# Daniel-Starr/pointcloudhookup

Hardware: AMD Instinct MI355X
Metric: Mpts/s ground-filter+tower-cluster, 100 M-pt corridor; % HBM roofline on kNN (higher is better)
Workload: dtype f32 (filter) + f64 (distance predicate)

## Files before the change

pointcloudhookup_amd/csrc/pch_dbscan.hip:

```cpp
#include <assert.h>
#include "pch_prims.h"

namespace pch {

constexpr int DB_THREADS = 256;
constexpr int DB_WAVES   = DB_THREADS / 64;
constexpr int DB_ROWS    = 25;
constexpr int INT_BIG    = 0x7fffffff;
constexpr int DB_FEW_QUERIES = 24;
constexpr int DB_AHEAD = 3;
constexpr long long DB_LONG_TOT = 8192;
constexpr int DB_SEGS = 43;

struct DbGrid {
    float   ox, oy, oz;
    double  cell;
    double  inv_cell;
    double  eps2;
    float   eps2_lo, eps2_hi;
    int     bx, by, bz;
    int     mx, my, mz;
    int64_t chunk_size;
    const uint32_t* chunk_bad;
    const uint32_t* chunk_cells;
    int     min_samples;
};

__constant__ int8_t DB_ROW_DY[DB_ROWS] = {0, 1, -1, 0, 0, 1, 1, -1, -1, 2, -2, 0, 0,
                                          2, 2, -2, -2, 1, 1, -1, -1, 2, 2, -2, -2};
__constant__ int8_t DB_ROW_DZ[DB_ROWS] = {0, 0, 0, 1, -1, 1, -1, 1, -1, 0, 0, 2, -2,
                                          1, -1, 1, -1, 2, -2, 2, -2, 2, -2, 2, -2};

__device__ __forceinline__ uint64_t db_pack(const DbGrid& g, uint64_t chunk, uint64_t cz,
                                            uint64_t cy, uint64_t cx) {
    return ((((chunk << g.bz) | cz) << g.by | cy) << g.bx) | cx;
}

__device__ __forceinline__ bool db_within(const float4& q, const float4& p, double eps2) {
    const double dx = (double)q.x - (double)p.x;
    const double dy = (double)q.y - (double)p.y;
    const double dz = (double)q.z - (double)p.z;
    double d = dx * dx;
    d += dy * dy;
    d += dz * dz;
    return d <= eps2;
}

__device__ __forceinline__ bool db_within2(const float4& q, const float4& p, const DbGrid& g) {
    const float dx = q.x - p.x, dy = q.y - p.y, dz = q.z - p.z;
    float d = dx * dx;
    d = __builtin_fmaf(dy, dy, d);
    d = __builtin_fmaf(dz, dz, d);
    if (d <= g.eps2_lo) return true;
    if (d >= g.eps2_hi) return false;
    return db_within(q, p, g.eps2);
}

typedef float f32x2 __attribute__((ext_vector_type(2)));
struct __attribute__((aligned(16))) DbPair { f32x2 x, y, z, pad; };

__device__ __forceinline__ void db_tile_put(DbPair* __restrict__ tile, int l, const float4& p) {
    float* f = reinterpret_cast<float*>(&tile[l >> 1]);
    f[l & 1] = p.x; f[2 + (l & 1)] = p.y; f[4 + (l & 1)] = p.z;
}
__device__ __forceinline__ float4 db_tile_get(const DbPair* __restrict__ tile, int k) {
    const float* f = reinterpret_cast<const float*>(&tile[k >> 1]);
    float4 p;
    p.x = f[k & 1]; p.y = f[2 + (k & 1)]; p.z = f[4 + (k & 1)]; p.w = 0.0f;
    return p;
}
__device__ __forceinline__ int db_tile_count(const float4& q, const DbPair* __restrict__ tile, int nj,
                                             const DbGrid& g) {
    const f32x2 qx = {q.x, q.x}, qy = {q.y, q.y}, qz = {q.z, q.z};
    const float lo = g.eps2_lo, hi = g.eps2_hi;
    int c_lo = 0, c_hi = 0;
    const int np = ((nj + 7) & ~7) >> 1;
    for (int k = 0; k < np; k += 4) {
        f32x2 px[4], py[4], pz[4];
#pragma unroll
        for (int u = 0; u < 4; ++u) { px[u] = tile[k + u].x; py[u] = tile[k + u].y; pz[u] = tile[k + u].z; }
#pragma unroll
        for (int u = 0; u < 4; ++u) {
            const f32x2 dx = qx - px[u], dy = qy - py[u], dz = qz - pz[u];
            f32x2 d = dx * dx;
            d = __builtin_elementwise_fma(dy, dy, d);
            d = __builtin_elementwise_fma(dz, dz, d);
            c_lo += (d.x <= lo ? 1 : 0) + (d.y <= lo ? 1 : 0);
            c_hi += (d.x < hi ? 1 : 0) + (d.y < hi ? 1 : 0);
        }
    }
    if (c_lo != c_hi) {
        c_lo = 0;
        for (int k = 0; k < nj; ++k) c_lo += db_within2(q, db_tile_get(tile, k), g) ? 1 : 0;
    }
    return c_lo;
}

__device__ __forceinline__ double db_box_d2(const float4& q, const float* __restrict__ box) {
    const double gx = fmax(fmax((double)box[0] - (double)q.x, (double)q.x - (double)box[3]), 0.0);
    const double gy = fmax(fmax((double)box[1] - (double)q.y, (double)q.y - (double)box[4]), 0.0);
    const double gz = fmax(fmax((double)box[2] - (double)q.z, (double)q.z - (double)box[5]), 0.0);
    double d = gx * gx;
    d += gy * gy;
    d += gz * gz;
    return d;
}
__device__ __forceinline__ double db_boxbox_d2(const float* __restrict__ a, const float* __restrict__ b) {
    const double gx = fmax(fmax((double)b[0] - (double)a[3], (double)a[0] - (double)b[3]), 0.0);
    const double gy = fmax(fmax((double)b[1] - (double)a[4], (double)a[1] - (double)b[4]), 0.0);
    const double gz = fmax(fmax((double)b[2] - (double)a[5], (double)a[2] - (double)b[5]), 0.0);
    double d = gx * gx;
    d += gy * gy;
    d += gz * gz;
    return d;
}

__device__ __forceinline__ bool db_row_bad(const float* __restrict__ xyz, int64_t i) {
    const uint32_t a = __float_as_uint(xyz[3 * i + 0]) & 0x7FFFFFFFu;
    const uint32_t b = __float_as_uint(xyz[3 * i + 1]) & 0x7FFFFFFFu;
    const uint32_t c = __float_as_uint(xyz[3 * i + 2]) & 0x7FFFFFFFu;
    return a >= 0x7F800000u || b >= 0x7F800000u || c >= 0x7F800000u;
}
__global__ __launch_bounds__(DB_THREADS) void db_chunkbad_k(const float* __restrict__ xyz, int64_t n,
                                                            int64_t chunk_size, uint32_t* __restrict__ bad) {
    for (int64_t i = (int64_t)blockIdx.x * DB_THREADS + threadIdx.x; i < n;
         i += (int64_t)gridDim.x * DB_THREADS)
        if (db_row_bad(xyz, i)) atomicOr(&bad[i / chunk_size], 1u);
}

__global__ __launch_bounds__(DB_THREADS) void db_first_bad_k(const float* __restrict__ xyz, int64_t n,
                                                             unsigned long long* __restrict__ first) {
    unsigned long long best = ~0ull;
    for (int64_t i = (int64_t)blockIdx.x * DB_THREADS + threadIdx.x; i < n;
         i += (int64_t)gridDim.x * DB_THREADS)
        if (db_row_bad(xyz, i) && (unsigned long long)i < best) best = (unsigned long long)i;
    best = wave_reduce_min(best);
    if (lane_id() == 0 && best != ~0ull) atomicMin(first, best);
}

__global__ __launch_bounds__(DB_THREADS) void db_aabb_in_k(const float* __restrict__ xyz, int64_t n,
                                                           uint32_t* __restrict__ mm) {
    uint32_t lo[3] = {0xFFFFFFFFu, 0xFFFFFFFFu, 0xFFFFFFFFu}, hi[3] = {0u, 0u, 0u};
    for (int64_t i = (int64_t)blockIdx.x * DB_THREADS + threadIdx.x; i < n;
         i += (int64_t)gridDim.x * DB_THREADS) {
        const float x = xyz[3 * i + 0], y = xyz[3 * i + 1], z = xyz[3 * i + 2];
        if (!(fabsf(x) < INFINITY && fabsf(y) < INFINITY && fabsf(z) < INFINITY)) continue;
        const float v[3] = {x, y, z};
#pragma unroll
        for (int a = 0; a < 3; ++a) {
            const uint32_t k = f32_ordered(v[a]);
            lo[a] = k < lo[a] ? k : lo[a];
            hi[a] = k > hi[a] ? k : hi[a];
        }
    }
#pragma unroll
    for (int a = 0; a < 3; ++a) {
        lo[a] = wave_reduce_min(lo[a]);
        hi[a] = wave_reduce_max(hi[a]);
        if (lane_id() == 0) {
            if (lo[a] != 0xFFFFFFFFu) atomicMin(&mm[a], lo[a]);
            if (hi[a] != 0u) atomicMax(&mm[3 + a], hi[a]);
        }
    }
}

__device__ __forceinline__ bool db_cell_coords(const DbGrid& g, float x, float y, float z,
                                               uint32_t& cx, uint32_t& cy, uint32_t& cz) {
    const double fx = floor(((double)x - (double)g.ox) * g.inv_cell);
    const double fy = floor(((double)y - (double)g.oy) * g.inv_cell);
    const double fz = floor(((double)z - (double)g.oz) * g.inv_cell);
    const bool ok = fx >= 0.0 && fx <= (double)g.mx && fy >= 0.0 && fy <= (double)g.my &&
                    fz >= 0.0 && fz <= (double)g.mz;
    cx = ok ? (uint32_t)fx : 0u; cy = ok ? (uint32_t)fy : 0u; cz = ok ? (uint32_t)fz : 0u;
    return ok;
}

__global__ __launch_bounds__(DB_THREADS) void db_keys_k(const float* __restrict__ xyz, int64_t n,
                                                        DbGrid g, const uint32_t* __restrict__ bad,
                                                        uint64_t* __restrict__ keys,
                                                        uint32_t* __restrict__ vals,
                                                        uint32_t* __restrict__ status) {
    const int64_t i = (int64_t)blockIdx.x * DB_THREADS + threadIdx.x;
    if (i >= n) return;
    vals[i] = (uint32_t)i;
    if (bad[i / g.chunk_size]) {
        keys[i] = db_pack(g, (uint64_t)(i / g.chunk_size), 0, 0, 0);
        return;
    }
    const float x = xyz[3 * i + 0], y = xyz[3 * i + 1], z = xyz[3 * i + 2];
    uint32_t cx, cy, cz;
    if (!db_cell_coords(g, x, y, z, cx, cy, cz)) atomicOr(status, 1u);
    keys[i] = db_pack(g, (uint64_t)(i / g.chunk_size), cz, cy, cx);
}

__global__ __launch_bounds__(DB_THREADS) void dbc_axis_keys_k(const float* __restrict__ xyz, int64_t n, int axis,
                                                              uint64_t* __restrict__ keys, uint32_t* __restrict__ vals) {
    const int64_t i = (int64_t)blockIdx.x * DB_THREADS + threadIdx.x;
    if (i >= n) return;
    keys[i] = f32_ordered(xyz[3 * i + axis]);
    vals[i] = (uint32_t)i;
}
__global__ __launch_bounds__(DB_THREADS) void dbc_heads_k(const uint64_t* __restrict__ keys, int64_t n, double inv_cell,
                                                          uint32_t* __restrict__ head) {
    const int64_t i = (int64_t)blockIdx.x * DB_THREADS + threadIdx.x;
    if (i >= n) return;
    bool h = i == 0;
    if (i > 0) {
        const double a = (double)f32_unordered((uint32_t)keys[i - 1]), b = (double)f32_unordered((uint32_t)keys[i]);
        h = (b - a) * inv_cell >= 3.0;
    }
    head[i] = h ? 1u : 0u;
}
__global__ __launch_bounds__(DB_THREADS) void dbc_local_k(const uint64_t* __restrict__ keys, const uint32_t* __restrict__ flag,
                                                          const uint32_t* __restrict__ excl, int64_t n, double inv_cell,
                                                          float* __restrict__ headx, int phase,
                                                          uint32_t* __restrict__ li, uint32_t* __restrict__ seglen,
                                                          uint32_t* __restrict__ status) {
    const int64_t i = (int64_t)blockIdx.x * DB_THREADS + threadIdx.x;
    if (i >= n) return;
    const uint32_t seg = excl[i] + flag[i] - 1u;
    const float x = f32_unordered((uint32_t)keys[i]);
    if (phase == 0) {
        if (flag[i]) headx[seg] = x;
        return;
    }
    const double v = floor(((double)x - (double)headx[seg]) * inv_cell);
    uint32_t u = 0;
    if (v >= 0.0 && v < 2147483000.0) u = (uint32_t)v; else atomicOr(status, 2u);
    li[i] = u;
    const bool last = i + 1 == n || flag[i + 1] != 0u;
    if (last) seglen[seg] = u + 3u;
}
__global__ __launch_bounds__(DB_THREADS) void dbc_comp_k(const uint32_t* __restrict__ vals, const uint32_t* __restrict__ flag,
                                                         const uint32_t* __restrict__ excl, const uint32_t* __restrict__ li,
                                                         const uint32_t* __restrict__ segoff, int64_t n, int axis,
                                                         uint32_t* __restrict__ comp, uint32_t* __restrict__ cmax) {
    const int64_t i = (int64_t)blockIdx.x * DB_THREADS + threadIdx.x;
    if (i >= n) return;
    const uint32_t seg = excl[i] + flag[i] - 1u;
    const uint32_t c = segoff[seg] + li[i];
    comp[3 * (int64_t)vals[i] + axis] = c;
    if (i == n - 1) cmax[axis] = c;
}
__global__ __launch_bounds__(DB_THREADS) void db_keys_comp_k(const uint32_t* __restrict__ comp, int64_t n, DbGrid g,
                                                             uint64_t* __restrict__ keys, uint32_t* __restrict__ vals) {
    const int64_t i = (int64_t)blockIdx.x * DB_THREADS + threadIdx.x;
    if (i >= n) return;
    vals[i] = (uint32_t)i;
    keys[i] = db_pack(g, 0, comp[3 * i + 2], comp[3 * i + 1], comp[3 * i + 0]);
}
__global__ __launch_bounds__(DB_THREADS) void db_add_offset_k(int32_t* __restrict__ labels, int64_t n, int32_t off) {
    const int64_t i = (int64_t)blockIdx.x * DB_THREADS + threadIdx.x;
    if (i < n && labels[i] >= 0) labels[i] += off;
}

__global__ __launch_bounds__(DB_THREADS) void db_gather_k(const float* __restrict__ xyz,
                                                          const uint64_t* __restrict__ keys,
                                                          const uint32_t* __restrict__ vals, int64_t n,
                                                          float4* __restrict__ pts) {
    const int64_t i = (int64_t)blockIdx.x * DB_THREADS + threadIdx.x;
    if (i >= n) return;
    const uint32_t o = vals[i];
    float4 p;
    p.x = xyz[3 * (int64_t)o + 0];
    p.y = xyz[3 * (int64_t)o + 1];
    p.z = xyz[3 * (int64_t)o + 2];
    p.w = __uint_as_float(o);
    pts[i] = p;
}

struct Row3 { float x, y, z; };
constexpr int CS_THREADS = 1024;
constexpr int CS_WAVES   = CS_THREADS / 64;
constexpr int CS_ROUNDS  = 4;
constexpr int CS_TILE    = CS_THREADS * CS_ROUNDS;
constexpr int CS_PASSES  = 4;
constexpr int CS_HREP    = 4;
constexpr int CS_BINS    = 512;
constexpr int64_t CS_MAX_CHUNK = 1 << 17;
constexpr int64_t CS_MIN_CHUNKS = 96;

__device__ __forceinline__ uint32_t cs_cell_key(const DbGrid& g, float x, float y, float z, bool& ok) {
    uint32_t cx, cy, cz;
    ok = db_cell_coords(g, x, y, z, cx, cy, cz);
    return (((cz << g.by) | cy) << g.bx) | cx;
}

constexpr int CS_HU = 8;
__device__ __forceinline__ void cs_load_rows(const Row3* __restrict__ rows, int i0, int cn, Row3 (&q)[CS_HU]) {
#pragma unroll
    for (int u = 0; u < CS_HU; ++u) {
        const int i = i0 + u * CS_THREADS + (int)threadIdx.x;
        q[u] = rows[i < cn ? i : 0];
    }
}
__device__ __forceinline__ bool cs_row_check(const Row3& q, bool in, bool ok, uint32_t* flags) {
    const bool fin = fabsf(q.x) < INFINITY && fabsf(q.y) < INFINITY && fabsf(q.z) < INFINITY;
    if (in && !fin) flags[0] = 1u;
    else if (in && !ok) flags[1] = 1u;
    return fin;
}
__device__ __forceinline__ uint64_t cs_chunk_field(const DbGrid& g, int64_t c) {
    const int sh = g.bx + g.by + g.bz;
    return sh < 64 ? ((uint64_t)c << sh) : 0ull;
}
__device__ __forceinline__ void cs_rows_in_place(const DbGrid& g, const Row3* __restrict__ rows, int cn, int64_t lo,
        uint64_t hi, bool isbad, float4* __restrict__ pts, uint64_t* __restrict__ keys_out) {
    for (int i = threadIdx.x; i < cn; i += CS_THREADS) {
        const Row3 q = rows[i];
        float4 o4;
        o4.x = q.x; o4.y = q.y; o4.z = q.z; o4.w = __uint_as_float((uint32_t)(lo + i));
        pts[lo + i] = o4;
        bool ok;
        if (keys_out) keys_out[lo + i] = isbad ? hi : (hi | cs_cell_key(g, q.x, q.y, q.z, ok));
// ... 329 lines not shown
    __syncthreads();
    for (int i0 = 0; i0 < cn; i0 += CS_HU * CS_THREADS) {
        Row3 q[CS_HU];
        cs_load_rows(rows, i0, cn, q);
#pragma unroll
        for (int u = 0; u < CS_HU; ++u) {
            const int i = i0 + u * CS_THREADS + tid;
            if (i < cn) {
                bool ok;
                const uint32_t k = cs_cell_key(g, q[u].x, q[u].y, q[u].z, ok);
                uint32_t h = ct_hash(k);
                for (int p = 0; p < CT_SLOTS && tkey[h] != k; ++p) h = (h + 1u) & (CT_SLOTS - 1);
                const uint32_t pos = atomicAdd(&tcnt[h], 1u);
                if (pos >= (uint32_t)cn) continue;
                float4 o4;
                o4.x = q[u].x; o4.y = q[u].y; o4.z = q[u].z; o4.w = __uint_as_float((uint32_t)(lo + i));
                pts[lo + pos] = o4;
                if constexpr (!TABLE) keys_out[lo + pos] = hi | k;
            }
        }
    }
}

constexpr int DC_ITEMS = SCAN_TILE / DB_THREADS;
static_assert(DC_ITEMS == 8, "two 64-byte key loads per thread");

__device__ __forceinline__ void dc_load_keys(const uint64_t* __restrict__ keys, int64_t base, int64_t n,
                                             uint64_t (&k)[DC_ITEMS], uint64_t& prev) {
    if (base + DC_ITEMS <= n) {
        const ulonglong2* q = reinterpret_cast<const ulonglong2*>(keys + base);
#pragma unroll
        for (int j = 0; j < DC_ITEMS / 2; ++j) { const ulonglong2 v = q[j]; k[2 * j] = v.x; k[2 * j + 1] = v.y; }
    } else {
#pragma unroll
        for (int j = 0; j < DC_ITEMS; ++j) k[j] = base + j < n ? keys[base + j] : 0ull;
    }
    prev = (base > 0 && base < n) ? keys[base - 1] : 0ull;
}

__global__ __launch_bounds__(DB_THREADS) void db_heads_k(const uint64_t* __restrict__ keys, int64_t n,
                                                         uint32_t* __restrict__ tile_sums) {
    __shared__ uint32_t wsum[DB_WAVES];
    const int64_t base = (int64_t)blockIdx.x * SCAN_TILE + (int64_t)threadIdx.x * DC_ITEMS;
    uint64_t k[DC_ITEMS], prev;
    dc_load_keys(keys, base, n, k, prev);
    uint32_t heads = 0;
#pragma unroll
    for (int j = 0; j < DC_ITEMS; ++j) {
        const int64_t i = base + j;
        heads += (i < n && (i == 0 || k[j] != (j ? k[j - 1] : prev))) ? 1u : 0u;
    }
    heads = wave_reduce_add(heads);
    if (lane_id() == 0) wsum[wave_id()] = heads;
    __syncthreads();
    if (threadIdx.x == 0) {
        uint32_t t = 0;
#pragma unroll
        for (int w = 0; w < DB_WAVES; ++w) t += wsum[w];
        tile_sums[blockIdx.x] = t;
    }
}

__global__ __launch_bounds__(DB_THREADS) void db_cells_k(const uint64_t* __restrict__ keys,
                                                         const uint32_t* __restrict__ tile_excl, int64_t n,
                                                         int sh, int64_t nchunks,
                                                         uint32_t* __restrict__ cid,
                                                         uint32_t* __restrict__ cell_start,
                                                         uint64_t* __restrict__ cell_key,
                                                         uint32_t* __restrict__ chunk_cells,
                                                         uint32_t* __restrict__ cell_acc) {
    __shared__ uint32_t wsum[DB_WAVES];
    const int64_t base = (int64_t)blockIdx.x * SCAN_TILE + (int64_t)threadIdx.x * DC_ITEMS;
    uint64_t k[DC_ITEMS], prev;
    dc_load_keys(keys, base, n, k, prev);
    bool hd[DC_ITEMS];
    uint32_t heads = 0;
#pragma unroll
    for (int j = 0; j < DC_ITEMS; ++j) {
        const int64_t i = base + j;
        hd[j] = i < n && (i == 0 || k[j] != (j ? k[j - 1] : prev));
        heads += hd[j] ? 1u : 0u;
    }
    const uint32_t incl = wave_scan_incl(heads);
    if (lane_id() == 63) wsum[wave_id()] = incl;
    __syncthreads();
    uint32_t c = tile_excl[blockIdx.x] + incl - heads;
    for (int w = 0; w < wave_id(); ++w) c += wsum[w];
    uint32_t cc[DC_ITEMS];
#pragma unroll
    for (int j = 0; j < DC_ITEMS; ++j) {
        const int64_t i = base + j;
        c += hd[j] ? 1u : 0u;
        cc[j] = c - 1u;
        if (hd[j]) {
            const uint64_t key = k[j], pk = j ? k[j - 1] : prev;
            cell_start[cc[j]] = (uint32_t)i;
            cell_key[cc[j]] = key;
            uint4* a4 = reinterpret_cast<uint4*>(cell_acc + 8 * (int64_t)cc[j]);
            a4[0] = make_uint4(0u, 0u, 0u, 0u);
            a4[1] = make_uint4(0u, 0u, 0u, 0u);
            const uint64_t ch = sh < 64 ? key >> sh : 0, pch = sh < 64 ? pk >> sh : 0;
            if (i == 0 || ch != pch) chunk_cells[ch] = cc[j];
        }
        if (i == n - 1) { cell_start[cc[j] + 1] = (uint32_t)n; chunk_cells[nchunks] = cc[j] + 1; }
    }
    if (base + DC_ITEMS <= n) {
        uint4* o = reinterpret_cast<uint4*>(cid + base);
        o[0] = make_uint4(cc[0], cc[1], cc[2], cc[3]);
        o[1] = make_uint4(cc[4], cc[5], cc[6], cc[7]);
    } else {
#pragma unroll
        for (int j = 0; j < DC_ITEMS; ++j)
            if (base + j < n) cid[base + j] = cc[j];
    }
}
constexpr int64_t DB_TABLE_MAX_CHUNKS = 16384;
constexpr int CC_THREADS = 1024;
constexpr int CC_ITEMS = (int)(DB_TABLE_MAX_CHUNKS / CC_THREADS);

__device__ __forceinline__ uint32_t ct_staged_cells(const uint32_t* __restrict__ ncell, int64_t c, int64_t cn) {
    const uint32_t v = ncell[c];
    return v < (uint32_t)cn ? v : (uint32_t)cn;
}

__global__ __launch_bounds__(CC_THREADS) void db_chunkcells_k(
    const uint32_t* __restrict__ ncell, const uint32_t* __restrict__ ovf, int nchunks, int64_t n, int64_t chunk_size,
    uint32_t* __restrict__ chunk_cells, uint32_t* __restrict__ cell_start, uint32_t* __restrict__ ncells,
    uint32_t* __restrict__ route) {
    __shared__ uint32_t wsum[CC_THREADS / 64];
    const int tid = threadIdx.x, c0 = tid * CC_ITEMS;
    uint32_t v[CC_ITEMS], sum = 0;
    int over = 0;
#pragma unroll
    for (int u = 0; u < CC_ITEMS; ++u) {
        const int c = c0 + u;
        v[u] = 0u;
        if (c < nchunks) {
            const int64_t lo = (int64_t)c * chunk_size;
            v[u] = ct_staged_cells(ncell, c, (n - lo) < chunk_size ? (n - lo) : chunk_size);
            over |= ovf[c] != 0u;
        }
        sum += v[u];
    }
    over = __syncthreads_or(over);
    const uint32_t incl = wave_scan_incl(sum);
    if (lane_id() == 63) wsum[wave_id()] = incl;
    __syncthreads();
    uint32_t run = incl - sum, total = 0;
    for (int w = 0; w < CC_THREADS / 64; ++w) { if (w < wave_id()) run += wsum[w]; total += wsum[w]; }
#pragma unroll
    for (int u = 0; u < CC_ITEMS; ++u) {
        if (c0 + u < nchunks) chunk_cells[c0 + u] = run;
        run += v[u];
    }
    if (tid == 0) {
        *route = over ? 1u : 0u;
        if (!over) {
            chunk_cells[nchunks] = total;
            cell_start[total] = (uint32_t)n;
            *ncells = total;
        }
    }
}

__global__ __launch_bounds__(DB_THREADS) void db_celltab_k(
    const uint32_t* __restrict__ route, DbStage st, const uint32_t* __restrict__ ovf,
    const uint32_t* __restrict__ chunk_cells, int64_t n, int64_t chunk_size, uint32_t* __restrict__ cid,
    uint32_t* __restrict__ cell_start, uint64_t* __restrict__ cell_key, uint32_t* __restrict__ cell_acc,
    uint64_t* __restrict__ keys_out) {
    const int64_t base = (int64_t)blockIdx.x * SCAN_TILE + (int64_t)threadIdx.x * DC_ITEMS;
    if (base >= n) return;
    const bool fill = *route != 0u;
    int64_t c = (uint32_t)base / (uint32_t)chunk_size;
    int64_t lo = c * chunk_size, end = lo + chunk_size < n ? lo + chunk_size : n;
    uint32_t nc = ct_staged_cells(st.ncell, c, end - lo), j = 0;
    for (uint32_t a = 1, b = nc; a < b;) {
        const uint32_t mid = a + (b - a) / 2;
        if (st.start[lo + mid] <= (uint32_t)base) { j = mid; a = mid + 1; } else b = mid;
    }
    int64_t next = j + 1 < nc ? (int64_t)st.start[lo + j + 1] : end;
    uint32_t cell0 = chunk_cells[c];
    bool skip = fill && ovf[c] != 0u;
    uint32_t cc[DC_ITEMS];
#pragma unroll
    for (int u = 0; u < DC_ITEMS; ++u) {
        const int64_t i = base + u;
        cc[u] = 0u;
        if (i >= n) continue;
        bool head = i == base && nc != 0u && (int64_t)st.start[lo + j] == i;
        if (i == end) {
            ++c; lo = end; end = lo + chunk_size < n ? lo + chunk_size : n;
            nc = ct_staged_cells(st.ncell, c, end - lo); j = 0;
            next = 1 < nc ? (int64_t)st.start[lo + 1] : end;
            cell0 = chunk_cells[c];
            skip = fill && ovf[c] != 0u;
            head = nc != 0u;
        } else if (i == next) {
            ++j;
            next = j + 1 < nc ? (int64_t)st.start[lo + j + 1] : end;
            head = true;
        }
        cc[u] = cell0 + j;
        if (fill) {
            if (!skip) keys_out[i] = st.key[lo + j];
        } else if (head) {
            cell_start[cc[u]] = (uint32_t)i;
            cell_key[cc[u]] = st.key[lo + j];
            uint4* a4 = reinterpret_cast<uint4*>(cell_acc + 8 * (int64_t)cc[u]);
            a4[0] = make_uint4(0u, 0u, 0u, 0u);
            a4[1] = make_uint4(0u, 0u, 0u, 0u);
        }
    }
    if (fill) return;
    if (base + DC_ITEMS <= n) {
        uint4* o = reinterpret_cast<uint4*>(cid + base);
        o[0] = make_uint4(cc[0], cc[1], cc[2], cc[3]);
        o[1] = make_uint4(cc[4], cc[5], cc[6], cc[7]);
    } else {
#pragma unroll
        for (int u = 0; u < DC_ITEMS; ++u)
            if (base + u < n) cid[base + u] = cc[u];
    }
}

struct RowSet {
    int ca[DB_ROWS], cb[DB_ROWS];
};

template <typename K>
__device__ __forceinline__ int db_lower(const K* __restrict__ a, int m, K k) {
    int lo = 0, hi = m;
    while (lo < hi) { const int mid = (lo + hi) >> 1; if (a[mid] < k) lo = mid + 1; else hi = mid; }
    return lo;
}
struct DbRowAt { int xlo, xhi, ny, nz; };
__device__ __forceinline__ bool db_row_at(const DbGrid& g, uint64_t key, int row, DbRowAt& at) {
    const uint64_t cx = key & ((1ull << g.bx) - 1);
    const uint64_t cy = (key >> g.bx) & ((1ull << g.by) - 1);
    const uint64_t cz = (key >> (g.bx + g.by)) & ((1ull << g.bz) - 1);
    at.ny = (int)cy + DB_ROW_DY[row];
    at.nz = (int)cz + DB_ROW_DZ[row];
    at.xlo = (int)cx - 2 < 0 ? 0 : (int)cx - 2;
    at.xhi = (int)cx + 2 > g.mx ? g.mx : (int)cx + 2;
    return at.ny >= 0 && at.ny <= g.my && at.nz >= 0 && at.nz <= g.mz;
}
template <typename K>
__device__ __forceinline__ int2 db_run_in(const K* __restrict__ a, int n, K klo, K khi) {
    int2 v;
    v.x = db_lower(a, n, klo);
    K kk[5];
#pragma unroll
    for (int i = 0; i < 5; ++i) kk[i] = v.x + i < n ? a[v.x + i] : ~K(0);
    int cntx = 0;
#pragma unroll
    for (int i = 0; i < 5; ++i) cntx += kk[i] <= khi ? 1 : 0;
    v.y = v.x + cntx;
    return v;
}
__device__ __forceinline__ int2 db_row_run(const DbGrid& g, const uint64_t* __restrict__ cell_key, uint64_t key,
                                           int row) {
    const int sh = g.bx + g.by + g.bz;
    const uint64_t chunk = sh < 64 ? (key >> sh) : 0;
    int2 v;
    v.x = 0; v.y = 0;
    DbRowAt at;
    if (db_row_at(g, key, row, at)) {
        const int c0 = (int)g.chunk_cells[chunk], c1 = (int)g.chunk_cells[chunk + 1];
        v = db_run_in(cell_key + c0, c1 - c0, db_pack(g, chunk, (uint64_t)at.nz, (uint64_t)at.ny, (uint64_t)at.xlo),
                      db_pack(g, chunk, (uint64_t)at.nz, (uint64_t)at.ny, (uint64_t)at.xhi));
        v.x += c0;
        v.y += c0;
    }
    return v;
}

__device__ __forceinline__ void db_rows(const DbGrid& g, const uint64_t* __restrict__ cell_key, uint64_t key,
                                        RowSet* __restrict__ rs, const int2* __restrict__ rowtab, int cell) {
    const int l = lane_id();
    if (rowtab) {
        if (l < DB_ROWS) {
            const int2 v = rowtab[(int64_t)cell * DB_ROWS + l];
            rs->ca[l] = v.x;
            rs->cb[l] = v.y;
        }
        __builtin_amdgcn_wave_barrier();
        return;
    }
    if (l < DB_ROWS) {
        const int2 v = db_row_run(g, cell_key, key, l);
        rs->ca[l] = v.x;
        rs->cb[l] = v.y;
    }
    __builtin_amdgcn_wave_barrier();
}

__global__ __launch_bounds__(DB_THREADS) void db_rowtab_k(DbGrid g, const uint64_t* __restrict__ cell_key,
                                                          int m, int2* __restrict__ rowtab) {
    const int c = (blockIdx.x * DB_WAVES + wave_id()) * 2 + (lane_id() >> 5);
    const int l = lane_id() & 31;
    if (c >= m || l >= DB_ROWS) return;
    rowtab[(int64_t)c * DB_ROWS + l] = db_row_run(g, cell_key, cell_key[c], l);
}

template <bool COUNT, int AHEAD>
__device__ __forceinline__ int db_query_sweep(const DbGrid& g, const float4* __restrict__ pts, const float4 qp,
                                              int count, int r, uint32_t j0, const uint32_t* sa, const uint32_t* sb,
                                              unsigned long long& n_useful, unsigned long long& n_slots) {
    const int l = lane_id();
    while (r < DB_SEGS && count < g.min_samples) {
        const uint32_t pb = sb[r];
        if (j0 >= pb) { ++r; if (r < DB_SEGS) j0 = sa[r]; continue; }
        float4 P[AHEAD];
#pragma unroll
        for (int u = 0; u < AHEAD; ++u) {
            const uint32_t j = j0 + 64u * u + l;
            P[u] = pts[j < pb ? j : pb - 1];
        }
#pragma unroll
        for (int u = 0; u < AHEAD; ++u) {
            const uint32_t jb = j0 + 64u * u;
            const bool hit = jb + l < pb && db_within2(qp, P[u], g);
            count += (int)__popcll(__ballot(hit));
            if (COUNT && jb < pb) { n_useful += (pb - jb) < 64u ? (pb - jb) : 64u; n_slots += 64; }
        }
        j0 += 64u * AHEAD;
    }
    return count;
}

template <bool COUNT>
__global__ __launch_bounds__(DB_THREADS) void db_core_k(DbGrid g, const float4* __restrict__ pts,
                                                        const uint32_t* __restrict__ cell_start,
                                                        const uint64_t* __restrict__ cell_key, int m,
                                                        const int2* __restrict__ rowtab,
                                                        uint8_t* __restrict__ core_s,
                                                        uint32_t* __restrict__ cell_ncore,
                                                        unsigned long long* __restrict__ stats) {
    unsigned long long n_useful = 0, n_slots = 0, n_tiles = 0;
    auto tally = [&]() {
        if (COUNT && lane_id() == 0) {
            atomicAdd(&stats[0], n_useful); atomicAdd(&stats[1], n_slots);
            atomicAdd(&stats[2], 1ull); atomicAdd(&stats[3], n_tiles);
        }
    };
    __shared__ RowSet rows[DB_WAVES];
    __shared__ DbPair tiles[DB_WAVES][32];
    __shared__ uint32_t seg_a[DB_WAVES][DB_SEGS], seg_b[DB_WAVES][DB_SEGS];
    const int c = blockIdx.x * DB_WAVES + wave_id();
    if (c >= m) return;
    const int l = lane_id();
    const uint32_t s = cell_start[c], e = cell_start[c + 1];
    const int cnt = (int)(e - s);
    {
        const int sh = g.bx + g.by + g.bz;
        if (g.chunk_bad[sh < 64 ? (cell_key[c] >> sh) : 0]) {
            for (uint32_t i = s + l; i < e; i += 64) core_s[i] = 0;
            if (l == 0) cell_ncore[c] = 0;
            return;
        }
    }
    if (cnt >= g.min_samples) {
        for (uint32_t i = s + l; i < e; i += 64) core_s[i] = 1;
        if (l == 0) cell_ncore[c] = (uint32_t)cnt;
        return;
    }
    RowSet* rs = &rows[wave_id()];
    db_rows(g, cell_key, cell_key[c], rs, rowtab, c);
    long long tot = 0;
    if (l < DB_ROWS) tot = (long long)cell_start[rs->cb[l]] - (long long)cell_start[rs->ca[l]];
    tot = wave_reduce_add(tot);
    if (tot < (long long)g.min_samples) {
        for (uint32_t i = s + l; i < e; i += 64) core_s[i] = 0;
        if (l == 0) cell_ncore[c] = 0;
        return;
    }
    uint32_t* sa = seg_a[wave_id()];
    uint32_t* sb = seg_b[wave_id()];
    {
        const uint64_t xmask = (1ull << g.bx) - 1;
        const int cx = (int)(cell_key[c] & xmask);
        if (l < DB_ROWS) {
            const int ca = rs->ca[l], cb = rs->cb[l];
            if (l < 9) {
                int ia = ca, ib = cb;
                if (ca < cb) {
                    if ((int)(cell_key[ca] & xmask) == cx - 2) ia = ca + 1;
                    if (ib > ia && (int)(cell_key[cb - 1] & xmask) == cx + 2) ib = cb - 1;
                }
                sa[l] = cell_start[ia];      sb[l] = cell_start[ib];
                sa[9 + l] = cell_start[ca];  sb[9 + l] = cell_start[ia];
                sa[18 + l] = cell_start[ib]; sb[18 + l] = cell_start[cb];
            } else {
                sa[18 + l] = cell_start[ca]; sb[18 + l] = cell_start[cb];
            }
        }
        __builtin_amdgcn_wave_barrier();
    }
    uint32_t ncore = 0;
    const bool long_sweep = tot >= DB_LONG_TOT;
    if (cnt < DB_FEW_QUERIES) {
        for (uint32_t q = s; q < e; ++q) {
            const float4 qp = pts[q];
            int count = 0;
            if (long_sweep) {
                for (int r = 0; r < DB_SEGS && count < g.min_samples; ++r) {
                    const uint32_t pa = sa[r], pb = sb[r];
                    for (uint32_t j0 = pa; j0 < pb && count < g.min_samples; j0 += 64u * DB_AHEAD) {
                        float4 P[DB_AHEAD];
#pragma unroll
                        for (int u = 0; u < DB_AHEAD; ++u) {
                            const uint32_t j = j0 + 64u * u + l;
                            P[u] = pts[j < pb ? j : pb - 1];
                        }
#pragma unroll
                        for (int u = 0; u < DB_AHEAD; ++u) {
                            const uint32_t jb = j0 + 64u * u;
                            const bool hit = jb + l < pb && db_within2(qp, P[u], g);
                            count += (int)__popcll(__ballot(hit));
                            if (COUNT && jb < pb) { n_useful += (pb - jb) < 64u ? (pb - jb) : 64u; n_slots += 64; }
                        }
                    }
                }
            } else {
                for (int r = 0; r < DB_SEGS && count < g.min_samples; ++r) {
                    const uint32_t pa = sa[r], pb = sb[r];
                    for (uint32_t j0 = pa; j0 < pb && count < g.min_samples; j0 += 64) {
                        const uint32_t j = j0 + l;
                        bool hit = false;
                        if (j < pb) hit = db_within2(qp, pts[j], g);
                        count += (int)__popcll(__ballot(hit));
                        if (COUNT) { n_useful += (pb - j0) < 64u ? (pb - j0) : 64u; n_slots += 64; }
                    }
                }
            }
            const bool is_core = count >= g.min_samples;
            if (l == 0) core_s[q] = is_core ? 1 : 0;
            ncore += is_core;
        }
        if (l == 0) cell_ncore[c] = ncore;
        tally();
        return;
    }
    DbPair* tile = tiles[wave_id()];
    for (uint32_t q0 = s; q0 < e; q0 += 64) {
        const bool valid = q0 + l < e;
        float4 Q;
        Q.x = Q.y = Q.z = 3.0e37f; Q.w = 0.0f;
        if (valid) Q = pts[q0 + l];
        int count = 0;
        unsigned long long active = __ballot(valid);
        int r = 0;
        uint32_t j0 = sa[0];
        while (r < DB_SEGS && __popcll(active) >= DB_FEW_QUERIES / 2) {
            const uint32_t pb = sb[r];
            if (j0 >= pb) { ++r; if (r < DB_SEGS) j0 = sa[r]; continue; }
            const int nj = (int)((pb - j0) < 64u ? (pb - j0) : 64u);
            float4 P;
            P.x = P.y = P.z = 3.0e38f; P.w = 0.0f;
            if (l < nj) P = pts[j0 + l];
            __builtin_amdgcn_wave_barrier();
            db_tile_put(tile, l, P);
            __builtin_amdgcn_wave_barrier();
            count += db_tile_count(Q, tile, nj, g);
            if (COUNT) {
                n_useful += (unsigned long long)__popcll(__ballot(valid)) * (unsigned)nj;
                n_slots += 64ull * (unsigned)((nj + 7) & ~7);
                ++n_tiles;
            }
            j0 += 64;
            active = __ballot(valid && count < g.min_samples);
        }
        while (active) {
            const int ql = (int)__builtin_ctzll(active);
            active &= active - 1;
            float4 qp;
            qp.x = __shfl(Q.x, ql, 64); qp.y = __shfl(Q.y, ql, 64); qp.z = __shfl(Q.z, ql, 64); qp.w = 0.0f;
            const int c0 = __shfl(count, ql, 64);
            const int cq = long_sweep
                ? db_query_sweep<COUNT, DB_AHEAD>(g, pts, qp, c0, r, j0, sa, sb, n_useful, n_slots)
                : db_query_sweep<COUNT, 1>(g, pts, qp, c0, r, j0, sa, sb, n_useful, n_slots);
            if (l == ql) count = cq;
        }
        const bool is_core = valid && count >= g.min_samples;
        if (valid) core_s[q0 + l] = is_core ? 1 : 0;
        ncore += (uint32_t)__popcll(__ballot(is_core));
    }
    if (l == 0) cell_ncore[c] = ncore;
    tally();
}

constexpr int DB_CS_ROUNDS = 16;

__device__ __forceinline__ void db_cellstats_flush(uint32_t* __restrict__ acc, uint32_t c, const uint32_t (&v)[7]) {
#pragma unroll
    for (int k = 0; k < 7; ++k)
        if (v[k]) atomicMax(&acc[8 * (int64_t)c + k], v[k]);
}

__global__ __launch_bounds__(DB_THREADS) void db_cellstats_k(const float4* __restrict__ pts,
                                                             const uint32_t* __restrict__ cid,
                                                             const uint8_t* __restrict__ core_s, int64_t n,
                                                             uint32_t* __restrict__ acc,
                                                             uint32_t* __restrict__ bits, int64_t nw) {
    {
        const int64_t t = (int64_t)blockIdx.x * DB_THREADS + threadIdx.x;
        if (t < nw) bits[t] = 0u;
    }
    const int64_t base = ((int64_t)blockIdx.x * DB_WAVES + wave_id()) * (64 * DB_CS_ROUNDS);
    if (base >= n) return;
    const int l = lane_id();
    constexpr uint32_t NONE = 0xFFFFFFFFu;
    uint32_t carry_c = NONE;
    uint32_t carry[7] = {0, 0, 0, 0, 0, 0, 0};
    uint32_t mine[7] = {0, 0, 0, 0, 0, 0, 0};
    auto fold_mine = [&]() {
#pragma unroll
        for (int k = 0; k < 7; ++k) {
            const uint32_t t = wave_reduce_max(mine[k]);
            carry[k] = t > carry[k] ? t : carry[k];
            mine[k] = 0;
        }
    };
    for (int r0 = 0; r0 < DB_CS_ROUNDS; r0 += 4) {
    if (base + r0 * 64 >= n) break;
    uint32_t c4[4], core4[4];
    float4 p4[4];
#pragma unroll
    for (int u = 0; u < 4; ++u) {
        const int64_t i = base + (r0 + u) * 64 + l;
        const bool in = i < n;
        c4[u] = in ? cid[i] : NONE - 1u;
        core4[u] = in ? core_s[i] : 0u;
        p4[u] = pts[in ? i : base];
    }
#pragma unroll
    for (int u = 0; u < 4; ++u) {
        const int64_t i = base + (r0 + u) * 64 + l;
        const bool in = i < n;
        const uint32_t c = c4[u];
        uint32_t v[7] = {0, 0, 0, 0, 0, 0, 0};
        if (core4[u]) {
            const float4 p = p4[u];
            const uint32_t kx = f32_ordered(p.x), ky = f32_ordered(p.y), kz = f32_ordered(p.z);
            v[0] = ~kx; v[1] = ~ky; v[2] = ~kz; v[3] = kx; v[4] = ky; v[5] = kz;
            v[6] = ~__float_as_uint(p.w);
        }
        if (__ballot(c != carry_c) == 0) {
#pragma unroll
            for (int k = 0; k < 7; ++k) mine[k] = v[k] > mine[k] ? v[k] : mine[k];
            continue;
        }
        if (carry_c != NONE) fold_mine();
#pragma unroll
        for (int o = 1; o < 64; o <<= 1) {
            const uint32_t cu = __shfl_up(c, o, 64);
            const bool same = l >= o && cu == c;
#pragma unroll
            for (int k = 0; k < 7; ++k) {
                const uint32_t t = __shfl_up(v[k], o, 64);
                if (same) v[k] = t > v[k] ? t : v[k];
            }
        }
        const uint32_t c0 = (uint32_t)__builtin_amdgcn_readlane((int)c, 0);
        if (carry_c != NONE) {
            if (carry_c == c0) {
                if (c == c0) {
#pragma unroll
                    for (int k = 0; k < 7; ++k) v[k] = carry[k] > v[k] ? carry[k] : v[k];
                }
            } else if (l == 0) {
                db_cellstats_flush(acc, carry_c, carry);
            }
        }
        const uint32_t cn = __shfl_down(c, 1, 64);
        const bool run_end = l == 63 || cn != c;
        if (run_end && l != 63 && in) db_cellstats_flush(acc, c, v);
        carry_c = (uint32_t)__builtin_amdgcn_readlane((int)c, 63);
        if (carry_c == NONE - 1u) carry_c = NONE;
#pragma unroll
        for (int k = 0; k < 7; ++k) carry[k] = (uint32_t)__builtin_amdgcn_readlane((int)v[k], 63);
    }
    }
    if (carry_c != NONE) {
        fold_mine();
        if (l == 0) db_cellstats_flush(acc, carry_c, carry);
    }
}

__device__ __forceinline__ int db_cell_decode(const uint32_t* __restrict__ acc, int64_t c, float (&box)[6]) {
    uint32_t a[7];
#pragma unroll
    for (int k = 0; k < 7; ++k) a[k] = acc[8 * c + k];
#pragma unroll
    for (int k = 0; k < 3; ++k) {
        box[k] = INFINITY;
        box[3 + k] = -INFINITY;
        if (a[k] != 0u) box[k] = f32_unordered(~a[k]);
        if (a[3 + k] != 0u) box[3 + k] = f32_unordered(a[3 + k]);
    }
    return a[6] != 0u ? (int)(~a[6]) : INT_BIG;
}

__global__ __launch_bounds__(DB_THREADS) void db_cellfin_k(const uint32_t* __restrict__ acc, int m,
                                                           float* __restrict__ cell_box,
                                                           int* __restrict__ cell_min,
                                                           int* __restrict__ parent,
                                                           int* __restrict__ comp_min) {
    const int c = blockIdx.x * DB_THREADS + threadIdx.x;
    if (c >= m) return;
    float box[6];
    const int mn = db_cell_decode(acc, c, box);
#pragma unroll
    for (int k = 0; k < 6; ++k) cell_box[6 * (int64_t)c + k] = box[k];
    cell_min[c] = mn;
    parent[c] = c;
    comp_min[c] = INT_BIG;
}

__device__ __forceinline__ float db_d2f(const float4& a, const float4& b) {
    const float dx = a.x - b.x, dy = a.y - b.y, dz = a.z - b.z;
    return __builtin_fmaf(dz, dz, __builtin_fmaf(dy, dy, dx * dx));
}
__device__ __forceinline__ float db_box_d2f(const float4& q, const float* __restrict__ box) {
    const float gx = fmaxf(fmaxf(box[0] - q.x, q.x - box[3]), 0.0f);
    const float gy = fmaxf(fmaxf(box[1] - q.y, q.y - box[4]), 0.0f);
    const float gz = fmaxf(fmaxf(box[2] - q.z, q.z - box[5]), 0.0f);
    return __builtin_fmaf(gz, gz, __builtin_fmaf(gy, gy, gx * gx));
}
template <typename F>
__device__ __forceinline__ int db_argmin(const float4* __restrict__ pts, const uint8_t* __restrict__ core_s,
                                         uint32_t s, uint32_t e, bool dense, F f) {
    const int l = lane_id();
    unsigned long long best = ~0ull;
    for (uint32_t i0 = s; i0 < e; i0 += 256) {
#pragma unroll
        for (int u = 0; u < 4; ++u) {
            const uint32_t i = i0 + 64 * u + l;
            if (i < e && (dense || core_s[i])) {
                const float d = f(pts[i]);
                const unsigned long long k = ((unsigned long long)__float_as_uint(d) << 32) | i;
                best = k < best ? k : best;
            }
        }
    }
    best = wave_reduce_min(best);
    return best == ~0ull ? -1 : (int)(uint32_t)best;
}

__device__ __forceinline__ bool db_cells_connected(const DbGrid& g, const float4* __restrict__ pts,
                                                   const uint8_t* __restrict__ core_s, uint32_t as, uint32_t ae,
                                                   bool a_dense, uint32_t bs, uint32_t be, bool b_dense,
                                                   const float* __restrict__ boxB, uint32_t a_from) {
    const int l = lane_id();
    if (ae - as > 64 || be - bs > 64) {
        int ia = db_argmin(pts, core_s, as, ae, a_dense, [&](const float4& p) { return db_box_d2f(p, boxB); });
        if (ia < 0) return false;
        float4 q = pts[ia];
        for (int it = 0; it < 3; ++it) {
            const int jb = db_argmin(pts, core_s, bs, be, b_dense, [&](const float4& p) { return db_d2f(q, p); });
            if (jb < 0) return false;
            const float4 pb = pts[jb];
            if (db_within2(q, pb, g)) return true;
            const int ia2 = db_argmin(pts, core_s, as, ae, a_dense, [&](const float4& p) { return db_d2f(p, pb); });
            const float4 pa = pts[ia2];
            if (db_within2(pa, pb, g)) return true;
            if (ia2 == ia) break;
            ia = ia2;
            q = pa;
        }
    }
    for (uint32_t a0 = a_from; a0 < ae; a0 += 64) {
        const uint32_t ia = a0 + l;
        float4 pa;
        pa.x = pa.y = pa.z = pa.w = 0.0f;
        bool near = false;
        if (ia < ae && (a_dense || core_s[ia])) {
            pa = pts[ia];
            near = !(db_box_d2(pa, boxB) > g.eps2);
        }
        unsigned long long todo = __ballot(near);
        while (todo) {
            const int src = (int)__builtin_ctzll(todo);
            todo &= todo - 1;
            float4 q;
            q.x = __shfl(pa.x, src, 64); q.y = __shfl(pa.y, src, 64); q.z = __shfl(pa.z, src, 64); q.w = 0.0f;
            for (uint32_t j0 = bs; j0 < be; j0 += 64) {
                const uint32_t j = j0 + l;
                bool hit = false;
                if (j < be && (b_dense || core_s[j])) hit = db_within2(q, pts[j], g);
                if (__ballot(hit)) return true;
            }
        }
    }
    return false;
}

__device__ __forceinline__ int uf_load(int* p) {
    return __hip_atomic_load(p, __ATOMIC_RELAXED, __HIP_MEMORY_SCOPE_AGENT);
}
__device__ __forceinline__ int uf_find(int* __restrict__ parent, int x) {
    int p = uf_load(&parent[x]);
    while (p != x) {
        const int gp = uf_load(&parent[p]);
        if (gp != p) __hip_atomic_store(&parent[x], gp, __ATOMIC_RELAXED, __HIP_MEMORY_SCOPE_AGENT);
        x = p;
        p = gp;
    }
    return x;
}
__device__ __forceinline__ void uf_union(int* __restrict__ parent, int a, int b) {
    for (;;) {
        a = uf_find(parent, a);
        b = uf_find(parent, b);
        if (a == b) return;
        if (a < b) { const int t = a; a = b; b = t; }
        const int old = atomicCAS(&parent[a], a, b);
        if (old == a) return;
        a = old;
    }
}

struct DbFace { int row; uint64_t want; };
__device__ __forceinline__ DbFace db_face(const DbGrid& g, uint64_t key, int dir) {
    return {dir == 1 ? 1 : 3, key + (dir == 0 ? 1ull : (dir == 1 ? (1ull << g.bx) : (1ull << (g.bx + g.by))))};
}
__device__ __forceinline__ bool db_link_open(const DbGrid& g, const float* __restrict__ cell_box,
                                             const float* __restrict__ boxB, const int* parent, int A, int B) {
    return parent[A] != parent[B] && !(db_boxbox_d2(cell_box + 6 * (int64_t)A, boxB) > g.eps2);
}

struct DbForest {
    const uint32_t* cell_start; const uint32_t* cell_ncore; const float* cell_box; int* parent;
};

__device__ __forceinline__ bool db_link_live(const DbGrid& g, const DbForest& f, int A, int B) {
    bool live = f.cell_ncore[B] != 0 && db_link_open(g, f.cell_box, f.cell_box + 6 * (int64_t)B, f.parent, A, B);
    if (live) live = uf_find(f.parent, A) != uf_find(f.parent, B);
    return live;
}

__device__ __forceinline__ void db_union_cell(const DbGrid& g, const float4* __restrict__ pts,
                                              const uint8_t* __restrict__ core_s, const DbForest& f, int A,
                                              const RowSet* rs, int* cd) {
    const int l = lane_id();
    int total;
    {
        int len = 0;
        if (l < DB_ROWS) { len = rs->cb[l] - rs->ca[l]; len = len < 0 ? 0 : len; }
        const int incl = wave_scan_incl(len);
        total = __shfl(incl, 63, 64);
        if (l < DB_ROWS)
            for (int k = 0; k < len; ++k) cd[incl - len + k] = rs->ca[l] + k;
    }
    __builtin_amdgcn_wave_barrier();
    const uint32_t as = f.cell_start[A], ae = f.cell_start[A + 1];
    const bool a_dense = f.cell_ncore[A] == (ae - as);
    for (int base = 0; base < total; base += 64) {
        int B = -1;
        if (base + l < total) B = cd[base + l];
        const bool live = B > A && db_link_live(g, f, A, B);
        unsigned long long todo = __ballot(live);
        while (todo) {
            const int src = (int)__builtin_ctzll(todo);
            todo &= todo - 1;
            const int Bs = __builtin_amdgcn_readlane(B, src);
            {
                int same = 0;
                if (l == 0) same = uf_find(f.parent, A) == uf_find(f.parent, Bs);
                if (__builtin_amdgcn_readfirstlane(same)) continue;
            }
            const uint32_t bs = f.cell_start[Bs], be = f.cell_start[Bs + 1];
            const bool b_dense = f.cell_ncore[Bs] == (be - bs);
            const float* boxB = f.cell_box + 6 * (int64_t)Bs;
            const bool connected = db_cells_connected(g, pts, core_s, as, ae, a_dense, bs, be, b_dense, boxB, as);
            if (connected && l == 0) uf_union(f.parent, A, Bs);
        }
    }
}

__global__ __launch_bounds__(DB_THREADS) void db_union_k(DbGrid g, const float4* __restrict__ pts,
                                                         const uint32_t* __restrict__ cell_start,
                                                         const uint64_t* __restrict__ cell_key, int m,
                                                         const int2* __restrict__ rowtab,
                                                         const uint8_t* __restrict__ core_s,
                                                         const uint32_t* __restrict__ cell_ncore,
// ... 1414 lines not shown
```

Baseline: 66080.

## Share neighbor loads across pending queries in DBSCAN core sweep

Replaces the per-query residual sweep with a pending-mask sweep. Each batch of neighbor points, up to AHEAD*DEPTH wavefronts of loads, is fetched once and tested against every still-unresolved query in the wave, instead of being reloaded for each query. The small-cell path (fewer than 24 queries) now goes through the same shared sweep rather than its own per-query loop. Also adds a f32 band test that falls back to f64 only near eps, 12-byte xyz loads, scalarized segment bounds and wave index, and lowers the long-sweep threshold. These cut repeated global loads, at the cost of more registers and lockstep loops over pending queries.

```diff
diff --git a/pointcloudhookup_amd/csrc/pch_dbscan.hip b/pointcloudhookup_amd/csrc/pch_dbscan.hip
--- a/pointcloudhookup_amd/csrc/pch_dbscan.hip
+++ b/pointcloudhookup_amd/csrc/pch_dbscan.hip
@@ -9,7 +9,8 @@
 constexpr int INT_BIG    = 0x7fffffff;
 constexpr int DB_FEW_QUERIES = 24;
 constexpr int DB_AHEAD = 3;
-constexpr long long DB_LONG_TOT = 8192;
+constexpr long long DB_LONG_TOT = 4096;
+constexpr int DB_DEPTH = 2;
 constexpr int DB_SEGS = 43;
 
 struct DbGrid {
@@ -945,28 +946,82 @@
     rowtab[(int64_t)c * DB_ROWS + l] = db_row_run(g, cell_key, cell_key[c], l);
 }
 
+typedef float f32x3 __attribute__((ext_vector_type(3)));
+__device__ __forceinline__ float4 db_load_xyz(const float4* __restrict__ p) {
+    const f32x3 v = *reinterpret_cast<const f32x3*>(p);
+    float4 r;
+    r.x = v.x; r.y = v.y; r.z = v.z; r.w = 0.0f;
+    return r;
+}
+
+__device__ __forceinline__ uint32_t db_seg(const uint32_t* seg, int r) {
+    return (uint32_t)__builtin_amdgcn_readfirstlane((int)seg[r]);
+}
+
+__device__ __forceinline__ bool db_within_sweep(const float4& q, const float4& p, const DbGrid& g) {
+    const float dx = q.x - p.x, dy = q.y - p.y, dz = q.z - p.z;
+    float d = dx * dx;
+    d = __builtin_fmaf(dy, dy, d);
+    d = __builtin_fmaf(dz, dz, d);
+    bool hit = d <= g.eps2_lo;
+    const bool band = !hit && d < g.eps2_hi;
+    if (__ballot(band)) {
+        float4 pp = p;
+        asm volatile("" : "+v"(pp.x), "+v"(pp.y), "+v"(pp.z));
+        if (band) hit = db_within(q, pp, g.eps2);
+    }
+    return hit;
+}
+
 template <bool COUNT, int AHEAD>
-__device__ __forceinline__ int db_query_sweep(const DbGrid& g, const float4* __restrict__ pts, const float4 qp,
-                                              int count, int r, uint32_t j0, const uint32_t* sa, const uint32_t* sb,
-                                              unsigned long long& n_useful, unsigned long long& n_slots) {
+__device__ __forceinline__ int db_pending_sweep(const DbGrid& g, const float4* __restrict__ pts, const float4 Q,
+                                                int count, unsigned long long& pending, int& r, uint32_t& j0,
+                                                const uint32_t* sa, const uint32_t* sb,
+                                                unsigned long long& n_useful, unsigned long long& n_slots) {
+    constexpr int DEPTH = AHEAD > 1 ? DB_DEPTH : 1;
+    constexpr int W = AHEAD * DEPTH;
     const int l = lane_id();
-    while (r < DB_SEGS && count < g.min_samples) {
-        const uint32_t pb = sb[r];
-        if (j0 >= pb) { ++r; if (r < DB_SEGS) j0 = sa[r]; continue; }
-        float4 P[AHEAD];
-#pragma unroll
-        for (int u = 0; u < AHEAD; ++u) {
-            const uint32_t j = j0 + 64u * u + l;
-            P[u] = pts[j < pb ? j : pb - 1];
-        }
-#pragma unroll
-        for (int u = 0; u < AHEAD; ++u) {
-            const uint32_t jb = j0 + 64u * u;
-            const bool hit = jb + l < pb && db_within2(qp, P[u], g);
-            count += (int)__popcll(__ballot(hit));
-            if (COUNT && jb < pb) { n_useful += (pb - jb) < 64u ? (pb - jb) : 64u; n_slots += 64; }
-        }
-        j0 += 64u * AHEAD;
+    while (r < DB_SEGS && pending) {
+        const uint32_t pb = db_seg(sb, r);
+        while (j0 < pb && pending) {
+            const float4* __restrict__ base = pts + j0;
+            const uint32_t left = pb - j0;
+            float4 P[W];
+#pragma unroll
+            for (int u = 0; u < W; ++u) {
+                const uint32_t o = 64u * u + (uint32_t)l;
+                if (64u * u < left) {
+                    const uint32_t ob = (o < left ? o : left - 1) << 4;
+                    P[u] = db_load_xyz(reinterpret_cast<const float4*>(reinterpret_cast<const char*>(base) + ob));
+                }
+            }
+#pragma unroll
+            for (int t = 0; t < DEPTH; ++t) {
+                if (t > 0 && (64u * AHEAD * t >= left || !pending)) break;
+                for (unsigned long long todo = pending; todo; todo &= todo - 1) {
+                    const int ql = (int)__builtin_ctzll(todo);
+                    float4 qp;
+                    qp.x = __int_as_float(__builtin_amdgcn_readlane(__float_as_int(Q.x), ql));
+                    qp.y = __int_as_float(__builtin_amdgcn_readlane(__float_as_int(Q.y), ql));
+                    qp.z = __int_as_float(__builtin_amdgcn_readlane(__float_as_int(Q.z), ql));
+                    qp.w = 0.0f;
+                    int hits = 0;
+#pragma unroll
+                    for (int u = t * AHEAD; u < (t + 1) * AHEAD; ++u) {
+                        const uint32_t jb = 64u * u;
+                        if (jb < left) {
+                            const bool hit = jb + (uint32_t)l < left && db_within_sweep(qp, P[u], g);
+                            hits += (int)__popcll(__ballot(hit));
+                            if (COUNT) { n_useful += (left - jb) < 64u ? (left - jb) : 64u; n_slots += 64; }
+                        }
+                    }
+                    if (l == ql) count += hits;
+                }
+                pending &= __ballot(count < g.min_samples);
+            }
+            j0 += 64u * W;
+        }
+        if (pending) { ++r; if (r < DB_SEGS) j0 = db_seg(sa, r); }
     }
     return count;
 }
@@ -989,7 +1044,8 @@
     __shared__ RowSet rows[DB_WAVES];
     __shared__ DbPair tiles[DB_WAVES][32];
     __shared__ uint32_t seg_a[DB_WAVES][DB_SEGS], seg_b[DB_WAVES][DB_SEGS];
-    const int c = blockIdx.x * DB_WAVES + wave_id();
+    const int wv = __builtin_amdgcn_readfirstlane((int)(threadIdx.x >> 6));
+    const int c = blockIdx.x * DB_WAVES + wv;
     if (c >= m) return;
     const int l = lane_id();
     const uint32_t s = cell_start[c], e = cell_start[c + 1];
@@ -1007,7 +1063,7 @@
         if (l == 0) cell_ncore[c] = (uint32_t)cnt;
         return;
     }
-    RowSet* rs = &rows[wave_id()];
+    RowSet* rs = &rows[wv];
     db_rows(g, cell_key, cell_key[c], rs, rowtab, c);
     long long tot = 0;
     if (l < DB_ROWS) tot = (long long)cell_start[rs->cb[l]] - (long long)cell_start[rs->ca[l]];
@@ -1017,8 +1073,8 @@
         if (l == 0) cell_ncore[c] = 0;
         return;
     }
-    uint32_t* sa = seg_a[wave_id()];
-    uint32_t* sb = seg_b[wave_id()];
+    uint32_t* sa = seg_a[wv];
+    uint32_t* sb = seg_b[wv];
     {
         const uint64_t xmask = (1ull << g.bx) - 1;
         const int cx = (int)(cell_key[c] & xmask);
@@ -1041,50 +1097,7 @@
     }
     uint32_t ncore = 0;
     const bool long_sweep = tot >= DB_LONG_TOT;
-    if (cnt < DB_FEW_QUERIES) {
-        for (uint32_t q = s; q < e; ++q) {
-            const float4 qp = pts[q];
-            int count = 0;
-            if (long_sweep) {
-                for (int r = 0; r < DB_SEGS && count < g.min_samples; ++r) {
-                    const uint32_t pa = sa[r], pb = sb[r];
-                    for (uint32_t j0 = pa; j0 < pb && count < g.min_samples; j0 += 64u * DB_AHEAD) {
-                        float4 P[DB_AHEAD];
-#pragma unroll
-                        for (int u = 0; u < DB_AHEAD; ++u) {
-                            const uint32_t j = j0 + 64u * u + l;
-                            P[u] = pts[j < pb ? j : pb - 1];
-                        }
-#pragma unroll
-                        for (int u = 0; u < DB_AHEAD; ++u) {
-                            const uint32_t jb = j0 + 64u * u;
-                            const bool hit = jb + l < pb && db_within2(qp, P[u], g);
-                            count += (int)__popcll(__ballot(hit));
-                            if (COUNT && jb < pb) { n_useful += (pb - jb) < 64u ? (pb - jb) : 64u; n_slots += 64; }
-                        }
-                    }
-                }
-            } else {
-                for (int r = 0; r < DB_SEGS && count < g.min_samples; ++r) {
-                    const uint32_t pa = sa[r], pb = sb[r];
-                    for (uint32_t j0 = pa; j0 < pb && count < g.min_samples; j0 += 64) {
-                        const uint32_t j = j0 + l;
-                        bool hit = false;
-                        if (j < pb) hit = db_within2(qp, pts[j], g);
-                        count += (int)__popcll(__ballot(hit));
-                        if (COUNT) { n_useful += (pb - j0) < 64u ? (pb - j0) : 64u; n_slots += 64; }
-                    }
-                }
-            }
-            const bool is_core = count >= g.min_samples;
-            if (l == 0) core_s[q] = is_core ? 1 : 0;
-            ncore += is_core;
-        }
-        if (l == 0) cell_ncore[c] = ncore;
-        tally();
-        return;
-    }
-    DbPair* tile = tiles[wave_id()];
+    DbPair* tile = tiles[wv];
     for (uint32_t q0 = s; q0 < e; q0 += 64) {
         const bool valid = q0 + l < e;
         float4 Q;
@@ -1093,37 +1106,31 @@
         int count = 0;
         unsigned long long active = __ballot(valid);
         int r = 0;
-        uint32_t j0 = sa[0];
-        while (r < DB_SEGS && __popcll(active) >= DB_FEW_QUERIES / 2) {
-            const uint32_t pb = sb[r];
-            if (j0 >= pb) { ++r; if (r < DB_SEGS) j0 = sa[r]; continue; }
-            const int nj = (int)((pb - j0) < 64u ? (pb - j0) : 64u);
-            float4 P;
-            P.x = P.y = P.z = 3.0e38f; P.w = 0.0f;
-            if (l < nj) P = pts[j0 + l];
-            __builtin_amdgcn_wave_barrier();
-            db_tile_put(tile, l, P);
-            __builtin_amdgcn_wave_barrier();
-            count += db_tile_count(Q, tile, nj, g);
-            if (COUNT) {
-                n_useful += (unsigned long long)__popcll(__ballot(valid)) * (unsigned)nj;
-                n_slots += 64ull * (unsigned)((nj + 7) & ~7);
-                ++n_tiles;
+        uint32_t j0 = db_seg(sa, 0);
+        if (cnt >= DB_FEW_QUERIES) {
+            while (r < DB_SEGS && __popcll(active) >= DB_FEW_QUERIES / 2) {
+                const uint32_t pb = db_seg(sb, r);
+                if (j0 >= pb) { ++r; if (r < DB_SEGS) j0 = db_seg(sa, r); continue; }
+                const int nj = (int)((pb - j0) < 64u ? (pb - j0) : 64u);
+                float4 P;
+                P.x = P.y = P.z = 3.0e38f; P.w = 0.0f;
+                if (l < nj) P = pts[j0 + l];
+                __builtin_amdgcn_wave_barrier();
+                db_tile_put(tile, l, P);
+                __builtin_amdgcn_wave_barrier();
+                count += db_tile_count(Q, tile, nj, g);
+                if (COUNT) {
+                    n_useful += (unsigned long long)__popcll(__ballot(valid)) * (unsigned)nj;
+                    n_slots += 64ull * (unsigned)((nj + 7) & ~7);
+                    ++n_tiles;
+                }
+                j0 += 64;
+                active = __ballot(valid && count < g.min_samples);
             }
-            j0 += 64;
-            active = __ballot(valid && count < g.min_samples);
-        }
-        while (active) {
-            const int ql = (int)__builtin_ctzll(active);
-            active &= active - 1;
-            float4 qp;
-            qp.x = __shfl(Q.x, ql, 64); qp.y = __shfl(Q.y, ql, 64); qp.z = __shfl(Q.z, ql, 64); qp.w = 0.0f;
-            const int c0 = __shfl(count, ql, 64);
-            const int cq = long_sweep
-                ? db_query_sweep<COUNT, DB_AHEAD>(g, pts, qp, c0, r, j0, sa, sb, n_useful, n_slots)
-                : db_query_sweep<COUNT, 1>(g, pts, qp, c0, r, j0, sa, sb, n_useful, n_slots);
-            if (l == ql) count = cq;
-        }
+        }
+        count = long_sweep
+            ? db_pending_sweep<COUNT, DB_AHEAD>(g, pts, Q, count, active, r, j0, sa, sb, n_useful, n_slots)
+            : db_pending_sweep<COUNT, 1>(g, pts, Q, count, active, r, j0, sa, sb, n_useful, n_slots);
         const bool is_core = valid && count >= g.min_samples;
         if (valid) core_s[q0 + l] = is_core ? 1 : 0;
         ncore += (uint32_t)__popcll(__ballot(is_core));
```

New measurement: 67860, median of 5. +2.7%, better.
